# neuphonic/neutts-air

Measured on AMD Instinct MI355X. Metric: codec-tokens/s, higher is better.
Workload: dtype bf16

## Files before the change

### neutts-air_amd/csrc/kapi.cpp

```cpp
#include <ntts/dev.h>

#include "../../include/neutts_hip.h"
#include "kernels/attn_prefill.h"
#include "kernels/gemm.h"
#include "kernels/gemv.h"
#include "kernels/norm.h"
#include "kernels/sample.h"
#include "kernels/score.h"

#include <string.h>

#include <vector>

using namespace ntts;

extern "C" int ntts_k_gemm_bf16(const void* A, int64_t lda, const void* W, const void* bias, void* C, int64_t ldc,
                                int32_t M, int32_t N, int32_t K, int32_t variant) {
    if (!A || !W || !C || M < 1 || N < 1 || K < 64 || (K % 64) || (lda % 8) || (ldc % 8)) return NTTS_EINVAL;
    GemmArgs a{};
    a.X = (const bf16_t*)A; a.ldx = lda; a.W = (const bf16_t*)W; a.ldw = K; a.bias = (const bf16_t*)bias;
    a.out = C; a.ldo = ldc; a.M = M; a.N = N; a.K = K;
    if (variant == 0) variant = M > 64 ? 1 : 2;
    if (variant == 1) NTTS_GEMM_L(EPI_BF16, a, 1, (hipStream_t)0);
    else if (variant == 2) NTTS_GEMM_S(EPI_BF16, a, 1, (hipStream_t)0);
    else if (variant == 4) NTTS_GEMM_XL(EPI_BF16, a, 1, (hipStream_t)0);
    else if (variant == 5) gemm_launch<4, 4, 4, EPI_BF16, 4, 0, 32>(a, 1, (hipStream_t)0);
    else if (variant == 6) gemm_launch<2, 2, 4, EPI_BF16, 3, 0, 32>(a, 1, (hipStream_t)0);
    else if (variant == 7) gemm_launch<4, 3, 4, EPI_BF16, 2, 0, 64, false, false, 6>(a, 1, (hipStream_t)0);
    else if (variant == 8) gemm_launch<4, 3, 5, EPI_BF16, 2>(a, 1, (hipStream_t)0);
    else if (variant == 9) gemm_launch<4, 2, 5, EPI_BF16, 2>(a, 1, (hipStream_t)0);
    else if (variant == 3) {
        if (bias || (N % 16) || ldc != N) return NTTS_EINVAL;
        const int ks = 4, ns = gemm_nsplit(K, ks);
        float* slabs = nullptr;
        if (hipMalloc((void**)&slabs, (size_t)ns * M * N * sizeof(float)) != hipSuccess) return NTTS_ENOMEM;
        a.out = slabs; a.ldo = N;
        NTTS_GEMM_S(EPI_SPLITK, a, ks, (hipStream_t)0);
        NormArgs n{};
        n.slabs = slabs; n.nslab = ns; n.slab_rows = M; n.resid_out = (bf16_t*)C; n.M = M; n.H = N;
        add_rmsnorm_launch(n, (hipStream_t)0);
        if (hipDeviceSynchronize() != hipSuccess) { hipFree(slabs); return NTTS_EHIP; }
        hipFree(slabs);
    } else return NTTS_EINVAL;
    if (hipDeviceSynchronize() != hipSuccess) return NTTS_EHIP;
    return hipGetLastError() == hipSuccess ? NTTS_OK : NTTS_EHIP;
}

NTTS_KERNEL(256) void fp8_quantize_kernel(const float* in, unsigned char* out, long n, float inv_scale) {
    const long i = ((long)blockIdx.x * 256 + threadIdx.x) * 2;
    if (i + 1 < n) { const unsigned short q = f2fp8x2(in[i] * inv_scale, in[i + 1] * inv_scale); out[i] = (unsigned char)(q & 0xff); out[i + 1] = (unsigned char)(q >> 8); }
    else if (i < n) out[i] = f2fp8c(in[i] * inv_scale);
}
extern "C" int ntts_k_fp8_quantize(const float* in_dev, void* out_dev, int64_t n, float inv_scale) {
    if (!in_dev || !out_dev || n < 1) return NTTS_EINVAL;
    NTTS_LAUNCH((fp8_quantize_kernel), dim3((unsigned)((n + 511) / 512)), dim3(256), (hipStream_t)0, in_dev, (unsigned char*)out_dev, (long)n, inv_scale);
    if (hipDeviceSynchronize() != hipSuccess) return NTTS_EHIP;
    return hipGetLastError() == hipSuccess ? NTTS_OK : NTTS_EHIP;
}
extern "C" int ntts_k_gemm_fp8(const void* A, const void* W, const float* wscale, float xscale, const void* bias, void* C,
                               int32_t M, int32_t N, int32_t K, int32_t variant) {
    if (!A || !W || !wscale || !C || M < 1 || N < 1 || K < 128 || (K % 128) || (N % 8)) return NTTS_EINVAL;
    GemmArgs a{};
    a.X = (const bf16_t*)A; a.ldx = K; a.W = (const bf16_t*)W; a.ldw = K; a.bias = (const bf16_t*)bias;
    a.out = C; a.ldo = N; a.M = M; a.N = N; a.K = K; a.wscale = wscale; a.xscale = xscale;
    if (variant == 2) gemm_launch<4, 1, 1, EPI_BF16, 4, 0, 64, false, true>(a, 1, (hipStream_t)0);
    else if (variant == 4) gemm_launch<4, 4, 4, EPI_BF16, 2, 0, 64, false, true>(a, 1, (hipStream_t)0);
    else gemm_launch<2, 2, 4, EPI_BF16, 2, 0, 64, false, true>(a, 1, (hipStream_t)0);
    if (hipDeviceSynchronize() != hipSuccess) return NTTS_EHIP;
    return hipGetLastError() == hipSuccess ? NTTS_OK : NTTS_EHIP;
}

extern "C" int ntts_k_rmsnorm_bf16(const void* x, const void* w, void* y, int32_t rows, int32_t cols, float eps) {
    if (!x || !w || !y || rows < 1 || cols < 8 || (cols % 8) || cols > 2048) return NTTS_EINVAL;
    NormArgs n{};
    n.o_bf16 = (const bf16_t*)x; n.norm_w = (const bf16_t*)w; n.normed_out = (bf16_t*)y; n.M = rows; n.H = cols; n.eps = eps;
    add_rmsnorm_launch(n, (hipStream_t)0);
    if (hipDeviceSynchronize() != hipSuccess) return NTTS_EHIP;
    return hipGetLastError() == hipSuccess ? NTTS_OK : NTTS_EHIP;
}

NTTS_KERNEL(256) void membw_copy_kernel(const u32x4* src, u32x4* dst, long n) {
    for (long i = (long)blockIdx.x * 256 + threadIdx.x; i < n; i += (long)gridDim.x * 256) dst[i] = src[i];
}

extern "C" int ntts_k_membw(size_t bytes, int32_t iters, double* gbps) {
    if (!gbps || bytes < 4096 || iters < 1) return NTTS_EINVAL;
    void *a = nullptr, *b = nullptr;
    if (hipMalloc(&a, bytes) != hipSuccess || hipMalloc(&b, bytes) != hipSuccess) { if (a) hipFree(a); return NTTS_ENOMEM; }
    hipMemset(a, 1, bytes);
    hipEvent_t e0, e1;
    hipEventCreate(&e0); hipEventCreate(&e1);
    const long n = bytes / 16;
    NTTS_LAUNCH((membw_copy_kernel), dim3(2048), dim3(256), (hipStream_t)0, (const u32x4*)a, (u32x4*)b, n);
    hipEventRecord(e0, 0);
    for (int i = 0; i < iters; ++i) NTTS_LAUNCH((membw_copy_kernel), dim3(2048), dim3(256), (hipStream_t)0, (const u32x4*)a, (u32x4*)b, n);
    hipEventRecord(e1, 0);
    hipEventSynchronize(e1);
    float ms = 0;
    hipEventElapsedTime(&ms, e0, e1);
    *gbps = ms > 0 ? 2.0 * (double)(n * 16) * iters / (ms * 1e-3) / 1e9 : 0;
    hipEventDestroy(e0); hipEventDestroy(e1);
    hipFree(a); hipFree(b);
    return hipDeviceSynchronize() == hipSuccess ? NTTS_OK : NTTS_EHIP;
}

NTTS_KERNEL(64) void empty_kernel(int* p) { if (p && threadIdx.x == 12345) *p = 0; }
NTTS_KERNEL(256) void prefetch_kernel(const u32x4* src, long n16, int* sink) {
    unsigned int acc = 0;
    for (long i = (long)blockIdx.x * 256 + threadIdx.x; i < n16; i += (long)gridDim.x * 256) acc ^= src[i][0];
    if (acc == 0x12345678u && sink) *sink = 1;
}

NTTS_KERNEL(256) void random_fill_kernel(bf16_t* dst, long n, unsigned int seed) {
    for (long i = (long)blockIdx.x * 256 + threadIdx.x; i < n; i += (long)gridDim.x * 256) {
        unsigned int h = (unsigned int)i * 0x9e3779b1u + seed;
        h ^= h >> 15; h *= 0x2c1b3c6du; h ^= h >> 12; h *= 0x297a2d39u; h ^= h >> 15;
        dst[i] = (bf16_t)(((h & 1u) << 15) | ((120u + ((h >> 1) & 7u)) << 7) | ((h >> 4) & 0x7fu));
    }
}

template <int WM, int WN, int TM, int NS, int BK = 64>
static void probe_launch(const GemmArgs& a, int ks, int abl) {
    constexpr int EPI = EPI_BF16;
    switch (abl) {
        case 1: gemm_launch<WM, WN, TM, EPI, NS, 1, BK>(a, ks, 0); break;
        case 2: gemm_launch<WM, WN, TM, EPI, NS, 2, BK>(a, ks, 0); break;
        case 3: gemm_launch<WM, WN, TM, EPI, NS, 3, BK>(a, ks, 0); break;
        case 4: gemm_launch<WM, WN, TM, EPI, NS, 4, BK>(a, ks, 0); break;
        case 7: gemm_launch<WM, WN, TM, EPI, NS, 7, BK>(a, ks, 0); break;
        default: gemm_launch<WM, WN, TM, EPI, NS, 0, BK>(a, ks, 0); break;
    }
}

static void probe_dispatch(int config, const GemmArgs& a, int ks, int abl) {
    switch (config) {
        case 0: NTTS_LAUNCH((empty_kernel), dim3(256), dim3(64), (hipStream_t)0, (int*)nullptr); break;
        case 10: probe_launch<4, 1, 1, 2>(a, ks, abl); break;
        case 11: probe_launch<4, 1, 1, 3>(a, ks, abl); break;
        case 12: probe_launch<4, 1, 1, 4>(a, ks, abl); break;
        case 13: probe_launch<4, 1, 1, 6>(a, ks, abl); break;
        case 20: probe_launch<2, 1, 1, 4>(a, ks, abl); break;
        case 21: probe_launch<2, 1, 2, 4>(a, ks, abl); break;
        case 22: probe_launch<1, 1, 4, 4>(a, ks, abl); break;
        case 23: probe_launch<2, 2, 2, 3>(a, ks, abl); break;
        case 24: probe_launch<4, 2, 1, 3>(a, ks, abl); break;
        case 25: probe_launch<8, 1, 1, 3>(a, ks, abl); break;
        case 26: probe_launch<4, 1, 2, 3>(a, ks, abl); break;
        case 30: probe_launch<2, 2, 4, 2>(a, ks, abl); break;
        case 31: probe_launch<2, 2, 4, 3>(a, ks, abl); break;
        case 40: probe_launch<4, 2, 4, 2>(a, ks, abl); break;
        case 41: probe_launch<2, 4, 4, 2>(a, ks, abl); break;
        case 42: probe_launch<4, 4, 4, 2>(a, ks, abl); break;
        case 43: probe_launch<4, 2, 4, 3>(a, ks, abl); break;
        case 44: probe_launch<2, 2, 8, 2>(a, ks, abl); break;
        case 45: probe_launch<2, 4, 8, 2>(a, ks, abl); break;
        case 46: probe_launch<4, 4, 4, 4, 32>(a, ks, abl); break;
        case 47: probe_launch<4, 4, 4, 3, 32>(a, ks, abl); break;
        case 48: probe_launch<2, 4, 8, 4, 32>(a, ks, abl); break;
        case 49: probe_launch<2, 2, 4, 4, 32>(a, ks, abl); break;
        case 50: probe_launch<4, 1, 4, 3>(a, ks, abl); break;
        case 51: probe_launch<8, 1, 2, 3>(a, ks, abl); break;
        case 52: probe_launch<8, 1, 2, 2>(a, ks, abl); break;
        case 53: probe_launch<8, 2, 2, 2>(a, ks, abl); break;
        case 54: probe_launch<4, 2, 2, 3>(a, ks, abl); break;
        case 55: probe_launch<4, 4, 5, 2>(a, ks, abl); break;
        case 57: probe_launch<2, 4, 10, 2>(a, ks, abl); break;
        case 58: probe_launch<2, 4, 12, 2>(a, ks, abl); break;
        case 59: probe_launch<4, 3, 5, 2>(a, ks, abl); break;
        case 60: probe_launch<4, 2, 5, 2>(a, ks, abl); break;
        case 56: probe_launch<4, 4, 6, 2>(a, ks, abl); break;
        default: break;
    }
}

extern "C" int ntts_k_gemm_probe(int32_t M, int32_t N, int32_t K, int32_t config, int32_t abl, int32_t copies, int32_t iters,
                                 double* us) {
    if (!us || M < 1 || N < 16 || K < 64 || (K % 64) || copies < 1 || iters < 1) return NTTS_EINVAL;
    bf16_t *X = nullptr, *W = nullptr, *C = nullptr;
    const size_t wn = (size_t)N * K;
    if (hipMalloc((void**)&X, (size_t)M * K * 2) != hipSuccess || hipMalloc((void**)&W, wn * 2 * copies) != hipSuccess ||
        hipMalloc((void**)&C, (size_t)M * N * 2) != hipSuccess)
        return NTTS_ENOMEM;
    hipMemset(X, 0x11, (size_t)M * K * 2);
    hipMemset(W, 0x22, wn * 2 * copies);
    if (abl & 32) {
        NTTS_LAUNCH((random_fill_kernel), dim3(2048), dim3(256), (hipStream_t)0, X, (long)M * K, 0x9e3779b9u);
        NTTS_LAUNCH((random_fill_kernel), dim3(2048), dim3(256), (hipStream_t)0, W, (long)(wn * copies), 0x85ebca6bu);
    }
    hipEvent_t e0, e1;
    hipEventCreate(&e0); hipEventCreate(&e1);
    const int ks = config >= 1000 ? config / 1000 : 1;
    config %= 1000;
    const bool pf = (abl & 8) != 0;
    const int tile_major = (abl & 16) ? 1 : 0;
    const bool x_ktm = (abl & 64) != 0;
    abl &= 7;
    auto run = [&](int i) {
        if (pf) NTTS_LAUNCH((prefetch_kernel), dim3(256), dim3(256), (hipStream_t)0, (const u32x4*)(W + (size_t)((i + 1) % copies) * wn), (long)(wn / 8), (int*)nullptr);
        GemmArgs a{};
        a.X = X; a.ldx = K; a.W = W + (size_t)(i % copies) * wn; a.ldw = K; a.out = C; a.ldo = N; a.M = M; a.N = N; a.K = K;
        a.w_tile_major = tile_major;
        if (x_ktm) { a.ldx = 64; a.x_kt_stride = (long)M * 128; }
        probe_dispatch(config, a, ks, abl);
    };
    for (int i = 0; i < copies && i < 8; ++i) run(i);
    hipEventRecord(e0, 0);
    for (int i = 0; i < iters; ++i) run(i);
    hipEventRecord(e1, 0);
    hipEventSynchronize(e1);
    float ms = 0;
    hipEventElapsedTime(&ms, e0, e1);
    *us = (double)ms * 1e3 / iters;
    hipEventDestroy(e0); hipEventDestroy(e1);
    hipFree(X); hipFree(W); hipFree(C);
    return hipDeviceSynchronize() == hipSuccess && hipGetLastError() == hipSuccess ? NTTS_OK : NTTS_EHIP;
}

NTTS_KERNEL(64) void mfma_probe_kernel(float* out) {
    const int l = lane_id(), g = l >> 4, c = l & 15;
    for (int probe = 0; probe < 3; ++probe) {
        bf16x8 a, b;
        for (int j = 0; j < 8; ++j) {
            float av, bv;
            if (probe == 0) { av = (g == 0 && j == 0) ? (float)c : 0.f; bv = (g == 0 && j == 0) ? 1.f : 0.f; }
            else if (probe == 1) { av = (g == 0 && j == 0) ? 1.f : 0.f; bv = (g == 0 && j == 0) ? (float)c : 0.f; }
            else { av = (float)(g * 8 + j + 1); bv = (g * 8 + j == (c * 2 + 1) % 32) ? 1.f : 0.f; }
            a[j] = (short)f2bf(av);
            b[j] = (short)f2bf(bv);
        }
        f32x4 d = {0.f, 0.f, 0.f, 0.f};
        d = mfma16(a, b, d);
        for (int r = 0; r < 4; ++r) out[(probe * 64 + l) * 4 + r] = d[r];
    }
}

NTTS_KERNEL(256) void chain_probe_kernel(int* sink) {
    if (threadIdx.x == 0 && sink[blockIdx.x & 1023] == 0x7fffffff) sink[0] = 1;
}
NTTS_KERNEL(256) void chain_touch_kernel(const u32x4* src, u32x4* dst) {
    const long i = (long)blockIdx.x * 256 + threadIdx.x;
    u32x4 v = src[i];
    v[0] += 1;
    dst[i] = v;
}
extern "C" int ntts_k_launch_chain_probe(int32_t n_kernels, int32_t grid, int32_t block, int32_t iters, double* us_per_chain) {
    if (!us_per_chain || n_kernels < 1 || n_kernels > 4096 || grid < 1 || (block != 256 && block != -256) || iters < 1) return NTTS_EINVAL;
    const bool touch = block < 0;
    block = 256;
    if (touch) {
        u32x4 *src = nullptr, *dst = nullptr;
        const size_t per = (size_t)grid * 256, total = per * n_kernels;
        hipStream_t st = nullptr; hipGraph_t g = nullptr; hipGraphExec_t ge = nullptr;
        if (hipMalloc((void**)&src, total * 16) != hipSuccess || hipMalloc((void**)&dst, per * 16) != hipSuccess) { hipFree(src); return NTTS_ENOMEM; }
        hipMemset(src, 1, total * 16);
        int rc = NTTS_EHIP;
        if (hipStreamCreateWithFlags(&st, hipStreamNonBlocking) == hipSuccess && hipStreamBeginCapture(st, hipStreamCaptureModeThreadLocal) == hipSuccess) {
            for (int i = 0; i < n_kernels; ++i) NTTS_LAUNCH((chain_touch_kernel), dim3(grid), dim3(256), st, (const u32x4*)(src + per * i), dst);
            if (hipStreamEndCapture(st, &g) == hipSuccess && g && hipGraphInstantiate(&ge, g, nullptr, nullptr, 0) == hipSuccess) {
                hipEvent_t e0, e1;
                hipEventCreate(&e0); hipEventCreate(&e1);
                for (int i = 0; i < 3; ++i) hipGraphLaunch(ge, st);
                hipEventRecord(e0, st);
                for (int i = 0; i < iters; ++i) hipGraphLaunch(ge, st);
                hipEventRecord(e1, st);
                if (hipEventSynchronize(e1) == hipSuccess) { float ms = 0; hipEventElapsedTime(&ms, e0, e1); *us_per_chain = (double)ms * 1e3 / iters; rc = NTTS_OK; }
                hipEventDestroy(e0); hipEventDestroy(e1);
            }
        }
        if (ge) hipGraphExecDestroy(ge);
        if (g) hipGraphDestroy(g);
        if (st) hipStreamDestroy(st);
        hipFree(src); hipFree(dst);
        (void)hipGetLastError();
        return rc;
    }
    int* sink = nullptr;
    hipStream_t st = nullptr;
    hipGraph_t g = nullptr;
    hipGraphExec_t ge = nullptr;
    if (hipMalloc((void**)&sink, 4096) != hipSuccess) return NTTS_ENOMEM;
    hipMemset(sink, 0, 4096);
    int rc = NTTS_EHIP;
    if (hipStreamCreateWithFlags(&st, hipStreamNonBlocking) == hipSuccess &&
        hipStreamBeginCapture(st, hipStreamCaptureModeThreadLocal) == hipSuccess) {
        for (int i = 0; i < n_kernels; ++i) NTTS_LAUNCH((chain_probe_kernel), dim3(grid), dim3(block), st, sink);
        if (hipStreamEndCapture(st, &g) == hipSuccess && g && hipGraphInstantiate(&ge, g, nullptr, nullptr, 0) == hipSuccess) {
            hipEvent_t e0, e1;
            hipEventCreate(&e0); hipEventCreate(&e1);
            for (int i = 0; i < 3; ++i) hipGraphLaunch(ge, st);
            hipEventRecord(e0, st);
            for (int i = 0; i < iters; ++i) hipGraphLaunch(ge, st);
            hipEventRecord(e1, st);
            if (hipEventSynchronize(e1) == hipSuccess) {
                float ms = 0;
                hipEventElapsedTime(&ms, e0, e1);
                *us_per_chain = (double)ms * 1e3 / iters;
                rc = NTTS_OK;
            }
            hipEventDestroy(e0); hipEventDestroy(e1);
        }
    }
    if (ge) hipGraphExecDestroy(ge);
    if (g) hipGraphDestroy(g);
    if (st) hipStreamDestroy(st);
    hipFree(sink);
    (void)hipGetLastError();
    return rc;
}

NTTS_KERNEL(256) void silu_probe_kernel(const bf16_t* in, bf16_t* out, long n, int variant) {
    const long i = (long)blockIdx.x * 256 + threadIdx.x;
    if (i >= n) return;
    if (variant == 2) {
        const float a = bf2f(in[i]), b = bf2f(in[(i ^ 1) < n ? (i ^ 1) : i]);
        if (a < -86.5f || b < -86.5f) out[i] = f2bf(silu_fast(a));
        else out[i] = f2bf(silu_fast2(f32x2{a, b})[0]);
        return;
    }
    out[i] = f2bf(variant ? silu_fast(bf2f(in[i])) : silu_f(bf2f(in[i])));
}
extern "C" int ntts_k_silu_probe(const void* in_bf16_dev, void* out_bf16_dev, int64_t n, int32_t variant) {
    if (!in_bf16_dev || !out_bf16_dev || n < 1) return NTTS_EINVAL;
// ... 428 lines not shown
```

### neutts-air_amd/csrc/kernels/gemm.h

```cpp
#pragma once
#include <ntts/dev.h>

namespace ntts {

enum GemmEpi {
    EPI_BF16 = 0,
    EPI_SILU_MUL = 1,
    EPI_SPLITK = 2,
    EPI_ARGMAX = 3,
    EPI_BF16_SILU = 4,
    EPI_F32 = 5,
    EPI_RESID = 6,
    EPI_SILU_SPLIT3 = 7,
    EPI_ARGMAX_PEN = 8,
    EPI_ARGMAX_LSE = 9,
    EPI_ARGMAX_PEN_LSE = 10,
    EPI_ARGMAX_LSE_TGT = 11
};
constexpr bool epi_is_argmax(int epi) { return epi == EPI_ARGMAX || epi == EPI_ARGMAX_PEN || epi == EPI_ARGMAX_LSE || epi == EPI_ARGMAX_PEN_LSE || epi == EPI_ARGMAX_LSE_TGT; }
constexpr bool epi_has_pen(int epi) { return epi == EPI_ARGMAX_PEN || epi == EPI_ARGMAX_PEN_LSE; }
constexpr bool epi_has_lse(int epi) { return epi == EPI_ARGMAX_LSE || epi == EPI_ARGMAX_PEN_LSE || epi == EPI_ARGMAX_LSE_TGT; }
constexpr bool epi_has_tgt(int epi) { return epi == EPI_ARGMAX_LSE_TGT; }

struct GemmArgs {
    const bf16_t* X;
    long ldx;
    const bf16_t* W;
    long ldw;
    int w_tile_major;
    const bf16_t* bias;
    const float* bias_f32;
    void* out;
    long ldo;
    int M, N, K;
    int k_tiles_per_split;
    int mblocks, nblocks;
    float* part_val;
    int* part_idx;
    int part_stride;
    const int* mask_eos;
    int eos_col1;
    float* logits;
    long ld_logits;
    bf16_t* logits_bf16;
    long ld_logits_bf16;
    const unsigned int* seen;
    long seen_pitch;
    const float* rep_pen;
    const float* resid;
    long ldr;
    const bf16_t* resid_bf16;
    long ldrb;
    const float* wscale;
    float xscale;
    float out_fp8_inv;
    int xcd_nsplit, xcd_per;
    int xcd_maffine, xcd_xps;
    long x_kt_stride;
    unsigned long long* tl;
    float* part_sum;
    const int* target;
    float* target_val;
};

NTTS_D void gemm_tile_from_linear(int t, int mblocks, int nblocks, int& mb, int& nb) {
    const int GM = 8;
    const int per_group = GM * nblocks;
    const int g = t / per_group;
    const int first_m = g * GM;
    const int gsz = (mblocks - first_m) < GM ? (mblocks - first_m) : GM;
    const int in = t - g * per_group;
    mb = first_m + in % gsz;
    nb = in / gsz;
}

NTTS_D void gemm_tile_coords(int bid, int mblocks, int nblocks, int& mb, int& nb) {
    const int ntiles = mblocks * nblocks;
    const int xcd = bid & 7, idx = bid >> 3;
    const int q = ntiles >> 3, r = ntiles & 7;
    const int t = (xcd < r ? xcd * (q + 1) : r * (q + 1) + (xcd - r) * q) + idx;
    const int GM = 8;
    const int per_group = GM * nblocks;
    const int g = t / per_group;
    const int first_m = g * GM;
    const int gsz = (mblocks - first_m) < GM ? (mblocks - first_m) : GM;
    const int in = t - g * per_group;
    mb = first_m + in % gsz;
    nb = in / gsz;
}

NTTS_D float silu_f(float x) { return x / (1.0f + fexp(-x)); }
NTTS_D float silu_fast(float x) {
    const float ax = __builtin_fminf(__builtin_fabsf(x), 126.0f);
    if (ax > 87.0f && x < 0.f) return silu_f(x);
    const float t = fexp2(-ax * 1.44269504088896340736f);
    const float r = frcp_refined(1.0f + t);
    return x * (x >= 0.f ? r : t * r);
}
typedef __attribute__((ext_vector_type(2))) float f32x2;
NTTS_D f32x2 silu_fast2(f32x2 x) {
    f32x2 ax;
    ax[0] = __builtin_fminf(__builtin_fabsf(x[0]), 126.0f);
    ax[1] = __builtin_fminf(__builtin_fabsf(x[1]), 126.0f);
    const f32x2 e = ax * -1.44269504088896340736f;
    f32x2 t;
    t[0] = fexp2(e[0]);
    t[1] = fexp2(e[1]);
    const f32x2 d = t + 1.0f;
    f32x2 r;
    r[0] = frcp_raw(d[0]);
    r[1] = frcp_raw(d[1]);
    r = __builtin_elementwise_fma(__builtin_elementwise_fma(-d, r, f32x2{1.0f, 1.0f}), r, r);
    const f32x2 tr = t * r;
    f32x2 sg;
    sg[0] = x[0] >= 0.f ? r[0] : tr[0];
    sg[1] = x[1] >= 0.f ? r[1] : tr[1];
    return x * sg;
}
NTTS_D float rep_penalised(float v, float pen) { return rbf(v < 0.f ? v * pen : v / pen); }
NTTS_D void lse_merge(float& mx, float& sum, float omx, float osum) {
    if (omx > mx) { sum = osum + sum * fexp(mx - omx); mx = omx; }
    else if (omx < mx) sum += osum * fexp(omx - mx);
    else sum += osum;
}
NTTS_D float gemm_bias(const GemmArgs& p, int n) { return p.bias_f32 ? p.bias_f32[n] : (p.bias ? bf2f(p.bias[n]) : 0.f); }

template <int TM, int EPI, int WN, bool F8 = false, bool F16 = false>
NTTS_D void gemm_epilogue(const GemmArgs& p, f32x4 (&acc)[TM][4], int mrow0, int n0, int wn, int nb, int split) {
    const int lane = lane_id();
    const int g = lane >> 4, l15 = lane & 15;
    const int nb16 = n0 + wn * 64 + g * 16;
    float sc[4][4];
    if constexpr (F8) {
#pragma unroll
        for (int j = 0; j < 4; ++j)
#pragma unroll
            for (int r = 0; r < 4; ++r) {
                const int n = nb16 + j * 4 + r;
                sc[j][r] = p.xscale * p.wscale[n < p.N ? n : p.N - 1];
            }
        if constexpr (EPI != EPI_BF16) {
#pragma unroll
            for (int a = 0; a < TM; ++a)
#pragma unroll
                for (int j = 0; j < 4; ++j)
#pragma unroll
                    for (int r = 0; r < 4; ++r) acc[a][j][r] *= sc[j][r];
        }
    }
#pragma unroll
    for (int a = 0; a < TM; ++a) {
        const int m = mrow0 + a * 16 + l15;
        const bool mok = m < p.M;
        if constexpr (EPI == EPI_BF16 || EPI == EPI_BF16_SILU) {
            alignas(16) bf16_t o[16];
#pragma unroll
            for (int j = 0; j < 4; ++j)
#pragma unroll
                for (int r = 0; r < 4; ++r) {
                    const int n = nb16 + j * 4 + r;
                    float v = acc[a][j][r];
                    if constexpr (F8 && EPI == EPI_BF16) v = __builtin_fmaf(v, sc[j][r], n < p.N ? gemm_bias(p, n) : 0.f);
                    else if (n < p.N) v += gemm_bias(p, n);
                    if constexpr (EPI == EPI_BF16_SILU) v = silu_fast(v);
                    o[j * 4 + r] = f2op<F16>(v);
                }
            if (mok) {
                bf16_t* dst = (bf16_t*)p.out + (long)m * p.ldo + nb16;
                if (nb16 + 16 <= p.N) {
                    *(u32x4*)dst = *(u32x4*)&o[0];
                    *(u32x4*)(dst + 8) = *(u32x4*)&o[8];
                } else {
                    for (int e = 0; e < 16; ++e)
                        if (nb16 + e < p.N) dst[e] = o[e];
                }
            }
        } else if constexpr (EPI == EPI_SILU_SPLIT3) {
            alignas(16) bf16_t hi[16], lo[16];
#pragma unroll
            for (int j = 0; j < 4; ++j)
#pragma unroll
                for (int r = 0; r < 4; ++r) {
                    const int n = nb16 + j * 4 + r;
                    float v = acc[a][j][r];
                    if (n < p.N) v += gemm_bias(p, n);
                    v = silu_fast(v);
                    hi[j * 4 + r] = f2bf(v);
                    lo[j * 4 + r] = f2bf(v - bf2f(hi[j * 4 + r]));
                }
            if (mok) {
                bf16_t* dst = (bf16_t*)p.out + (long)m * p.ldo + nb16;
                if (nb16 + 16 <= p.N) {
                    *(u32x4*)dst = *(u32x4*)&hi[0];
                    *(u32x4*)(dst + 8) = *(u32x4*)&hi[8];
                    *(u32x4*)(dst + p.N) = *(u32x4*)&lo[0];
                    *(u32x4*)(dst + p.N + 8) = *(u32x4*)&lo[8];
                    *(u32x4*)(dst + 2 * p.N) = *(u32x4*)&hi[0];
                    *(u32x4*)(dst + 2 * p.N + 8) = *(u32x4*)&hi[8];
                } else {
                    for (int e = 0; e < 16; ++e)
                        if (nb16 + e < p.N) { dst[e] = hi[e]; dst[p.N + e] = lo[e]; dst[2 * p.N + e] = hi[e]; }
                }
            }
        } else if constexpr (EPI == EPI_RESID) {
            if (mok) {
                const bf16_t* rs = p.resid_bf16 + (long)m * p.ldrb + nb16;
                bf16_t* dst = (bf16_t*)p.out + (long)m * p.ldo + nb16;
                if (nb16 + 16 <= p.N) {
                    alignas(16) bf16_t rr[16], o[16];
                    *(u32x4*)&rr[0] = *(const u32x4*)rs;
                    *(u32x4*)&rr[8] = *(const u32x4*)(rs + 8);
#pragma unroll
                    for (int j = 0; j < 4; ++j)
#pragma unroll
                        for (int r = 0; r < 4; ++r)
                            o[j * 4 + r] = f2bf(bf2f(rr[j * 4 + r]) + rbf(acc[a][j][r] + gemm_bias(p, nb16 + j * 4 + r)));
// ... 157 lines not shown
                p.part_idx[pi] = bidx;
                if constexpr (epi_has_lse(EPI)) p.part_sum[pi] = lsum;
            }
        }
    }
}

template <int TM, int TN, int EPI, int WN>
NTTS_D void gemm_epilogue_nat(const GemmArgs& p, f32x4 (&acc)[TM][TN], int mrow0, int nw0, int wn, int nb) {
    const int lane = lane_id();
    const int g = lane >> 4, l15 = lane & 15;
#pragma unroll
    for (int a = 0; a < TM; ++a) {
        const int m = mrow0 + a * 16 + l15;
        const bool mok = m < p.M;
        if constexpr (EPI == EPI_BF16) {
#pragma unroll
            for (int j = 0; j < TN; ++j) {
                const int n4 = nw0 + j * 16 + g * 4;
                alignas(8) bf16_t o[4];
#pragma unroll
                for (int r = 0; r < 4; ++r) o[r] = f2bf(acc[a][j][r] + (n4 + r < p.N ? gemm_bias(p, n4 + r) : 0.f));
                if (mok) {
                    bf16_t* dst = (bf16_t*)p.out + (long)m * p.ldo + n4;
                    if (n4 + 4 <= p.N) *(u32x2*)dst = *(u32x2*)&o[0];
                    else for (int e = 0; e < 4; ++e) if (n4 + e < p.N) dst[e] = o[e];
                }
            }
        } else if constexpr (epi_is_argmax(EPI)) {
            float best = -INFINITY;
            int bidx = 0x7fffffff;
            const int meos = (mok && p.mask_eos) ? p.mask_eos[m] : 0;
            if constexpr (epi_has_pen(EPI)) {
                static_assert(TN % 2 == 0, "whole bitmap words per wave tile");
                const float pen = mok ? p.rep_pen[m] : 1.0f;
                unsigned int sw[TN / 2], any = 0;
#pragma unroll
                for (int q = 0; q < TN / 2; ++q) sw[q] = 0;
                if (pen != 1.0f) {
                    const unsigned int* sp = p.seen + (long)m * p.seen_pitch + (nw0 >> 5);
#pragma unroll
                    for (int q = 0; q < TN / 2; ++q) { sw[q] = sp[q]; any |= sw[q]; }
                }
                if (any) {
#pragma unroll
                    for (int j = 0; j < TN; ++j)
#pragma unroll
                        for (int r = 0; r < 4; ++r)
                            if ((sw[j >> 1] >> ((j & 1) * 16 + g * 4 + r)) & 1u) acc[a][j][r] = rep_penalised(rbf(acc[a][j][r]), pen);
                }
            }
            int tgt = -1;
            if constexpr (epi_has_tgt(EPI)) { if (mok) tgt = p.target[m]; }
#pragma unroll
            for (int j = 0; j < TN; ++j) {
                alignas(8) bf16_t lo[4];
#pragma unroll
                for (int r = 0; r < 4; ++r) {
                    const int n = nw0 + j * 16 + g * 4 + r;
                    float v = rbf(acc[a][j][r]);
                    if (meos && n == (p.eos_col1 > 0 ? p.eos_col1 - 1 : meos - 1)) v = -INFINITY;
                    lo[r] = f2bf(v);
                    if constexpr (epi_has_tgt(EPI)) { if (n == tgt) p.target_val[m] = v; }
                    if (n < p.N) {
                        if (mok && p.logits) p.logits[(long)m * p.ld_logits + n] = v;
                        if (v > best) { best = v; bidx = n; }
                    }
                    if constexpr (epi_has_lse(EPI)) acc[a][j][r] = n < p.N ? v : -INFINITY;
                }
                if (p.logits_bf16 && mok) {
                    const int n4 = nw0 + j * 16 + g * 4;
                    bf16_t* dst = p.logits_bf16 + (long)m * p.ld_logits_bf16 + n4;
                    if (n4 + 4 <= p.N) *(u32x2*)dst = *(u32x2*)&lo[0];
                    else for (int e = 0; e < 4; ++e) if (n4 + e < p.N) dst[e] = lo[e];
                }
            }
            float lsum = 0.f;
            if constexpr (epi_has_lse(EPI)) {
                if (best > -INFINITY) {
#pragma unroll
                    for (int j = 0; j < TN; ++j)
#pragma unroll
                        for (int r = 0; r < 4; ++r) lsum += fexp(acc[a][j][r] - best);
                }
            }
#pragma unroll
            for (int sh = 16; sh <= 32; sh <<= 1) {
                const float ov = shfl_xor(best, sh);
                const int oi = shfl_xor(bidx, sh);
                if constexpr (epi_has_lse(EPI)) {
                    const float os = shfl_xor(lsum, sh);
                    float mx = best;
                    lse_merge(mx, lsum, ov, os);
                }
                if (ov > best || (ov == best && oi < bidx)) { best = ov; bidx = oi; }
            }
            if (mok && g == 0) {
                const long pi = (long)m * p.part_stride + nb * WN + wn;
                p.part_val[pi] = best;
                p.part_idx[pi] = bidx;
                if constexpr (epi_has_lse(EPI)) p.part_sum[pi] = lsum;
            }
        } else {
            static_assert(epi_is_argmax(EPI) || EPI == EPI_BF16, "epilogues of the natural-order tile");
        }
    }
}

template <int WM, int WN, int TM, int EPI, int NS, int ABL = 0, int BK = 64, bool WNT = false, bool F8 = false, int TN = 4, bool F16 = false>
NTTS_KERNEL(WM * WN * 64) void gemm_kernel(GemmArgs p) {
    static_assert(!F16 || (!F8 && TN == 4 && (EPI == EPI_BF16 || EPI == EPI_BF16_SILU || EPI == EPI_F32)), "fp16 operands: codec GEMMs");
    static_assert(BK == 64 || BK == 32, "ring slot K extent");
    static_assert(!F8 || BK == 64, "fp8: one ring slot = 128-byte rows");
    static_assert(TN == 4 || ((epi_is_argmax(EPI) || EPI == EPI_BF16) && !F8 && BK == 64), "natural-order tile: lm_head / prefill QKV, bf16");
    constexpr int ESZ = F8 ? 1 : 2;
    constexpr int CW = TN * 16;
    constexpr int BM = WM * TM * 16, BN = WN * CW, NW = WM * WN;
    constexpr int ROWS = BM + BN;
    constexpr int KC = BK / 8;
    constexpr int RPI = 64 / KC;
    static_assert(ROWS % RPI == 0, "whole loader instructions");
    constexpr int NINST = ROWS / RPI;
    constexpr int SPT = 64 / BK;
    constexpr int PER_WAVE = (NINST + NW - 1) / NW;
    constexpr bool EVEN = NINST % NW == 0;
    static_assert(NS >= 2 && (NS - 2) * PER_WAVE <= 63, "vmcnt range");
    NTTS_SHARED bf16_t lds[NS * ROWS * BK];
    auto swz = [](int rho) { return BK == 64 ? (rho >> 1) & 7 : (rho >> 2) & 3; };

    const int lane = lane_id(), wave = wave_id();
    const int wm = wave / WN, wn = wave % WN;
    const int g = lane >> 4, l15 = lane & 15;
    int mb, nb, split = blockIdx.y;
    if (p.xcd_maffine > 0) {
        const int xcd = blockIdx.x & 7, j = blockIdx.x >> 3;
        const int wi = (xcd % p.xcd_xps) + p.xcd_xps * j;
        if (wi >= p.nblocks * p.xcd_maffine) return;
        mb = xcd / p.xcd_xps;
        nb = wi % p.nblocks;
        split = wi / p.nblocks;
    } else if (p.xcd_nsplit) {
        const int xcd = blockIdx.x & 7, j = blockIdx.x >> 3, xps = 8 / p.xcd_nsplit;
        split = xcd / xps;
        const int t = (xcd % xps) * p.xcd_per + j;
        if (t >= p.mblocks * p.nblocks) return;
        gemm_tile_from_linear(t, p.mblocks, p.nblocks, mb, nb);
    } else {
        gemm_tile_coords(blockIdx.x, p.mblocks, p.nblocks, mb, nb);
    }
    const long tlb = ((long)blockIdx.y * gridDim.x + blockIdx.x) * 16;
    auto mark = [&](int slot) { if (p.tl && wave == 0 && lane == 0) p.tl[tlb + slot] = now_ticks(); };
    mark(0);
    const int m0 = mb * BM, n0 = nb * BN;
    const int ktiles = F8 ? p.K >> 7 : p.K >> 6;
    const int kt0 = split * p.k_tiles_per_split * SPT;
    int nk = ktiles - split * p.k_tiles_per_split;
    if (nk > p.k_tiles_per_split) nk = p.k_tiles_per_split;
    nk *= SPT;

    const char* src[PER_WAVE];
#pragma unroll
    for (int i = 0; i < PER_WAVE; ++i) {
        const int inst = (EVEN || wave + i * NW < NINST) ? wave + i * NW : 0;
        const int rho = inst * RPI + lane / KC;
        const int c = (lane % KC) ^ swz(rho);
        if (rho < BM) {
            int m = m0 + rho;
            if (m > p.M - 1) m = p.M - 1;
            src[i] = (const char*)p.X + (long)m * p.ldx * ESZ + c * 16;
        } else {
            const int q = rho - BM;
            const int wq = q >> 6, j = (q >> 4) & 3, i16 = q & 15;
            int n = TN == 4 ? n0 + wq * 64 + (i16 >> 2) * 16 + j * 4 + (i16 & 3) : n0 + q;
            if (n > p.N - 1) n = p.N - 1;
            src[i] = p.w_tile_major ? (const char*)p.W + (long)(n >> 6) * 64 * p.K * ESZ + (n & 63) * 128 + c * 16
                                    : (const char*)p.W + (long)n * p.ldw * ESZ + c * 16;
        }
    }
    const long xstep = p.x_kt_stride > 0 ? p.x_kt_stride : BK * 2;
    const long wstep = p.w_tile_major ? 8192 : xstep;
    auto stage = [&](int kt, int buf) {
        if constexpr (ABL & 2) return;
#pragma unroll
        for (int i = 0; i < PER_WAVE; ++i) {
            const int inst = wave + i * NW;
            if (!EVEN && inst >= NINST) continue;
            const bool is_w = (inst * RPI) >= BM;
            const char* g = src[i] + (long)(kt0 + kt) * (is_w ? wstep : xstep);
            bf16_t* l = lds + buf * (ROWS * BK) + inst * 512;
            if (WNT && is_w) glds16_nt(g, l); else glds16(g, l);
        }
    };

    f32x4 acc[TM][TN];
#pragma unroll
    for (int a = 0; a < TM; ++a)
#pragma unroll
        for (int j = 0; j < TN; ++j) acc[a][j] = f32x4{0.f, 0.f, 0.f, 0.f};

    int xoff[TM], woff[TN], xsw[TM], wsw[TN];
#pragma unroll
    for (int a = 0; a < TM; ++a) {
        const int rho = wm * TM * 16 + a * 16 + l15;
        xoff[a] = rho * BK;
        xsw[a] = swz(rho);
    }
#pragma unroll
    for (int j = 0; j < TN; ++j) {
        const int rho = BM + wn * CW + j * 16 + l15;
        woff[j] = rho * BK;
        wsw[j] = swz(rho);
    }
    const bool full_share = EVEN || wave + (PER_WAVE - 1) * NW < NINST;

#pragma unroll
    for (int s = 0; s < NS - 1; ++s)
        if (s < nk) stage(s, s);
    mark(1);
    int buf = 0;
    for (int kt = 0; kt < nk; ++kt) {
        if (kt + NS - 2 < nk) {
            if (full_share) wait_vmem_le<(NS - 2) * PER_WAVE>(); else wait_vmem_le<(NS - 2) * (PER_WAVE - 1)>();
        } else wait_vmem();
        sync_keep_dma();
        if (kt == 0) mark(2);
        if (kt + NS - 1 < nk) stage(kt + NS - 1, buf == 0 ? NS - 1 : buf - 1);
        const bf16_t* base = lds + buf * (ROWS * BK);
        buf = buf + 1 == NS ? 0 : buf + 1;
        if constexpr (ABL & 1) continue;
#pragma unroll
        for (int ks = 0; ks < BK / 32; ++ks) {
            const int c = ks * 4 + g;
            bf16x8 xb[TM], wa[TN];
#pragma unroll
            for (int a = 0; a < TM; ++a) xb[a] = ld16<bf16x8>(base + xoff[a] + ((c ^ xsw[a]) << 3));
#pragma unroll
            for (int j = 0; j < TN; ++j) wa[j] = ld16<bf16x8>(base + woff[j] + ((c ^ wsw[j]) << 3));
#pragma unroll
            for (int a = 0; a < TM; ++a)
#pragma unroll
                for (int j = 0; j < TN; ++j) {
                    if constexpr (F8) {
                        const i64x2 w2 = __builtin_bit_cast(i64x2, wa[j]), x2 = __builtin_bit_cast(i64x2, xb[a]);
                        acc[a][j] = mfma16_fp8(w2[0], x2[0], acc[a][j]);
                        acc[a][j] = mfma16_fp8(w2[1], x2[1], acc[a][j]);
                    } else {
                        acc[a][j] = mfma16_op<F16>(wa[j], xb[a], acc[a][j]);
                    }
                }
        }
    }

    if constexpr (ABL & 4) {
        if (acc[0][0][0] != 12345.678f) return;
    }
    if (p.tl && wave == 0 && lane == 0) p.tl[tlb + 3] = now_ticks() + (acc[0][0][0] == 1.2345e30f ? 1 : 0);
    if constexpr (TN == 4) gemm_epilogue<TM, EPI, WN, F8, F16>(p, acc, m0 + wm * TM * 16, n0, wn, nb, split);
    else gemm_epilogue_nat<TM, TN, EPI, WN>(p, acc, m0 + wm * TM * 16, n0 + wn * CW, wn, nb);
    if (p.tl) { mark(4); wait_vmem(); mark(5); }
}





struct GemmShape { int BM, BN, WN; };

template <int WM, int WN, int TM, int EPI, int NS = 2, int ABL = 0, int BK = 64, bool WNT = false, bool F8 = false, int TN = 4, bool F16 = false>
inline void gemm_launch(GemmArgs p, int ksplit, hipStream_t s) {
    constexpr int BM = WM * TM * 16, BN = WN * TN * 16;
    p.mblocks = (p.M + BM - 1) / BM;
    p.nblocks = (p.N + BN - 1) / BN;
    const int ktiles = p.K / (F8 ? 128 : 64);
    if (ksplit < 1) ksplit = 1;
    if (ksplit > ktiles) ksplit = ktiles;
    p.k_tiles_per_split = (ktiles + ksplit - 1) / ksplit;
    const int nsplit = (ktiles + p.k_tiles_per_split - 1) / p.k_tiles_per_split;
    if constexpr (epi_is_argmax(EPI)) p.part_stride = p.nblocks * WN;
    if (EPI == EPI_SPLITK && p.xcd_maffine == -1 && (p.mblocks == 1 || p.mblocks == 2 || p.mblocks == 4 || p.mblocks == 8)) {
        p.xcd_maffine = nsplit;
        p.xcd_xps = 8 / p.mblocks;
        p.xcd_nsplit = 0;
        const int per_xcd = (p.nblocks * nsplit + p.xcd_xps - 1) / p.xcd_xps;
        NTTS_LAUNCH((gemm_kernel<WM, WN, TM, EPI, NS, ABL, BK, WNT, F8, TN, F16>), dim3(8 * per_xcd), dim3(WM * WN * 64), s, p);
        return;
    }
    p.xcd_maffine = 0;
    if (EPI == EPI_SPLITK && p.xcd_nsplit == -1 && (nsplit == 2 || nsplit == 4 || nsplit == 8)) {
        p.xcd_nsplit = nsplit;
        const int xps = 8 / nsplit, tiles = p.mblocks * p.nblocks;
        p.xcd_per = (tiles + xps - 1) / xps;
        NTTS_LAUNCH((gemm_kernel<WM, WN, TM, EPI, NS, ABL, BK, WNT, F8, TN, F16>), dim3(8 * p.xcd_per), dim3(WM * WN * 64), s, p);
        return;
    }
    p.xcd_nsplit = 0;
    NTTS_LAUNCH((gemm_kernel<WM, WN, TM, EPI, NS, ABL, BK, WNT, F8, TN, F16>), dim3(p.mblocks * p.nblocks, nsplit), dim3(WM * WN * 64), s, p);
}

#define NTTS_GEMM_XL(EPI, p, ks, s) ::ntts::gemm_launch<4, 4, 4, EPI, 2>(p, ks, s)
#define NTTS_GEMM_BIG(EPI, p, s) do { \
    const long txl_ = (long)(((p).M + 255) / 256) * (((p).N + 255) / 256), tl_ = (long)(((p).M + 127) / 128) * (((p).N + 127) / 128); \
    if ((p).N >= 256 && txl_ >= 140) NTTS_GEMM_XL(EPI, p, 1, s); else if (tl_ >= 240) NTTS_GEMM_L(EPI, p, 1, s); else NTTS_GEMM_S(EPI, p, 1, s); } while (0)
#define NTTS_GEMM_L(EPI, p, ks, s) ::ntts::gemm_launch<2, 2, 4, EPI, 2>(p, ks, s)
#define NTTS_GEMM_BIG_F16(EPI, p, s) do { \
    const long txl_ = (long)(((p).M + 255) / 256) * (((p).N + 255) / 256), tl_ = (long)(((p).M + 127) / 128) * (((p).N + 127) / 128); \
    if ((p).N >= 256 && txl_ >= 140) ::ntts::gemm_launch<4, 4, 4, EPI, 2, 0, 64, false, false, 4, true>(p, 1, s); \
    else if (tl_ >= 240) ::ntts::gemm_launch<2, 2, 4, EPI, 2, 0, 64, false, false, 4, true>(p, 1, s); \
    else ::ntts::gemm_launch<4, 1, 1, EPI, 4, 0, 64, false, false, 4, true>(p, 1, s); } while (0)
#define NTTS_GEMM_S(EPI, p, ks, s) ::ntts::gemm_launch<4, 1, 1, EPI, 4>(p, ks, s)

template <int EPI>
inline void lm_head_launch_epi(const GemmArgs& a, int head_tile, bool fp8, hipStream_t s) {
    switch (head_tile) {
        case 0:
            if (fp8) gemm_launch<4, 1, 1, EPI, 4, 0, 64, false, true>(a, 1, s);
            else gemm_launch<4, 1, 1, EPI, 4>(a, 1, s);
            break;
        case 4: gemm_launch<4, 3, 4, EPI, 2, 0, 64, true, false, 6>(a, 1, s); break;
        case 3: gemm_launch<4, 3, 5, EPI, 2, 0, 64, true>(a, 1, s); break;
        case 2:
            if (fp8) gemm_launch<4, 4, 4, EPI, 2, 0, 64, true, true>(a, 1, s);
            else gemm_launch<4, 4, 4, EPI, 2, 0, 64, true>(a, 1, s);
            break;
        default:
            if (fp8) gemm_launch<2, 2, 4, EPI, 2, 0, 64, false, true>(a, 1, s);
            else gemm_launch<2, 2, 4, EPI, 2>(a, 1, s);
    }
}
inline void lm_head_launch(const GemmArgs& a, int head_tile, bool fp8, hipStream_t s) {
    if (a.target) {
        lm_head_launch_epi<EPI_ARGMAX_LSE_TGT>(a, head_tile, fp8, s);
    } else if (a.part_sum) {
        if (a.seen) lm_head_launch_epi<EPI_ARGMAX_PEN_LSE>(a, head_tile, fp8, s);
        else lm_head_launch_epi<EPI_ARGMAX_LSE>(a, head_tile, fp8, s);
    } else if (a.seen) lm_head_launch_epi<EPI_ARGMAX_PEN>(a, head_tile, fp8, s);
    else lm_head_launch_epi<EPI_ARGMAX>(a, head_tile, fp8, s);
}
inline long seen_pitch_for(int N) { return ((long)N + 288 + 31) / 32 / 4 * 4 + 4; }

inline int gemm_nsplit(int K, int ksplit, int ktile = 64) {
    const int ktiles = K / ktile;
    if (ksplit < 1) ksplit = 1;
    if (ksplit > ktiles) ksplit = ktiles;
    const int per = (ktiles + ksplit - 1) / ksplit;
    return (ktiles + per - 1) / per;
}

}
```

Before: 186,400.

## Use half-width tile specialization for last N block in XL GEMM

For the 4x4x4 XL GEMM configuration, blocks covering the final 128 or fewer columns of N run a specialized path. Each wave computes a 32-row by 64-column sub-tile over only half the W columns, and stages one fewer load per wave, so no work is wasted on out-of-range columns. The compute body is rewrapped in a generic lambda templated on tile rows and loads per wave. A new variant 10 and extra probe configs allow disabling the path or comparing against it. It adds code size and register pressure, and it assumes the LDS layout still matches when fewer instructions are staged.

```diff
diff --git a/neutts-air_amd/csrc/kapi.cpp b/neutts-air_amd/csrc/kapi.cpp
--- a/neutts-air_amd/csrc/kapi.cpp
+++ b/neutts-air_amd/csrc/kapi.cpp
@@ -29,6 +29,7 @@
     else if (variant == 7) gemm_launch<4, 3, 4, EPI_BF16, 2, 0, 64, false, false, 6>(a, 1, (hipStream_t)0);
     else if (variant == 8) gemm_launch<4, 3, 5, EPI_BF16, 2>(a, 1, (hipStream_t)0);
     else if (variant == 9) gemm_launch<4, 2, 5, EPI_BF16, 2>(a, 1, (hipStream_t)0);
+    else if (variant == 10) { a.no_half_block = 1; NTTS_GEMM_XL(EPI_BF16, a, 1, (hipStream_t)0); }
     else if (variant == 3) {
         if (bias || (N % 16) || ldc != N) return NTTS_EINVAL;
         const int ks = 4, ns = gemm_nsplit(K, ks);
@@ -119,16 +120,16 @@
     }
 }
 
-template <int WM, int WN, int TM, int NS, int BK = 64>
+template <int WM, int WN, int TM, int NS, int BK = 64, int TN = 4>
 static void probe_launch(const GemmArgs& a, int ks, int abl) {
     constexpr int EPI = EPI_BF16;
     switch (abl) {
-        case 1: gemm_launch<WM, WN, TM, EPI, NS, 1, BK>(a, ks, 0); break;
-        case 2: gemm_launch<WM, WN, TM, EPI, NS, 2, BK>(a, ks, 0); break;
-        case 3: gemm_launch<WM, WN, TM, EPI, NS, 3, BK>(a, ks, 0); break;
-        case 4: gemm_launch<WM, WN, TM, EPI, NS, 4, BK>(a, ks, 0); break;
-        case 7: gemm_launch<WM, WN, TM, EPI, NS, 7, BK>(a, ks, 0); break;
-        default: gemm_launch<WM, WN, TM, EPI, NS, 0, BK>(a, ks, 0); break;
+        case 1: gemm_launch<WM, WN, TM, EPI, NS, 1, BK, false, false, TN>(a, ks, 0); break;
+        case 2: gemm_launch<WM, WN, TM, EPI, NS, 2, BK, false, false, TN>(a, ks, 0); break;
+        case 3: gemm_launch<WM, WN, TM, EPI, NS, 3, BK, false, false, TN>(a, ks, 0); break;
+        case 4: gemm_launch<WM, WN, TM, EPI, NS, 4, BK, false, false, TN>(a, ks, 0); break;
+        case 7: gemm_launch<WM, WN, TM, EPI, NS, 7, BK, false, false, TN>(a, ks, 0); break;
+        default: gemm_launch<WM, WN, TM, EPI, NS, 0, BK, false, false, TN>(a, ks, 0); break;
     }
 }
 
@@ -168,6 +169,8 @@
         case 58: probe_launch<2, 4, 12, 2>(a, ks, abl); break;
         case 59: probe_launch<4, 3, 5, 2>(a, ks, abl); break;
         case 60: probe_launch<4, 2, 5, 2>(a, ks, abl); break;
+        case 61: probe_launch<4, 3, 4, 2>(a, ks, abl); break;
+        case 62: probe_launch<4, 3, 4, 2, 64, 6>(a, ks, abl); break;
         case 56: probe_launch<4, 4, 6, 2>(a, ks, abl); break;
         default: break;
     }
diff --git a/neutts-air_amd/csrc/kernels/gemm.h b/neutts-air_amd/csrc/kernels/gemm.h
--- a/neutts-air_amd/csrc/kernels/gemm.h
+++ b/neutts-air_amd/csrc/kernels/gemm.h
@@ -61,7 +61,9 @@
     float* part_sum;
     const int* target;
     float* target_val;
+    int no_half_block;
 };
+template <int V> struct gemm_ic { static constexpr int value = V; };
 
 NTTS_D void gemm_tile_from_linear(int t, int mblocks, int nblocks, int& mb, int& nb) {
     const int GM = 8;
@@ -525,6 +527,9 @@
     auto mark = [&](int slot) { if (p.tl && wave == 0 && lane == 0) p.tl[tlb + slot] = now_ticks(); };
     mark(0);
     const int m0 = mb * BM, n0 = nb * BN;
+    constexpr bool HALF_OK = WM == 4 && WN == 4 && TM == 4 && TN == 4 && BK == 64 && !F8 && !epi_is_argmax(EPI);
+    bool half = false;
+    if constexpr (HALF_OK) half = !p.no_half_block && n0 + 128 >= p.N;
     const int ktiles = F8 ? p.K >> 7 : p.K >> 6;
     const int kt0 = split * p.k_tiles_per_split * SPT;
     int nk = ktiles - split * p.k_tiles_per_split;
@@ -552,10 +557,10 @@
     }
     const long xstep = p.x_kt_stride > 0 ? p.x_kt_stride : BK * 2;
     const long wstep = p.w_tile_major ? 8192 : xstep;
-    auto stage = [&](int kt, int buf) {
+    auto stage = [&](int kt, int buf, auto npw_) {
         if constexpr (ABL & 2) return;
 #pragma unroll
-        for (int i = 0; i < PER_WAVE; ++i) {
+        for (int i = 0; i < decltype(npw_)::value; ++i) {
             const int inst = wave + i * NW;
             if (!EVEN && inst >= NINST) continue;
             const bool is_w = (inst * RPI) >= BM;
@@ -565,73 +570,81 @@
         }
     };
 
-    f32x4 acc[TM][TN];
-#pragma unroll
-    for (int a = 0; a < TM; ++a)
-#pragma unroll
-        for (int j = 0; j < TN; ++j) acc[a][j] = f32x4{0.f, 0.f, 0.f, 0.f};
-
-    int xoff[TM], woff[TN], xsw[TM], wsw[TN];
-#pragma unroll
-    for (int a = 0; a < TM; ++a) {
-        const int rho = wm * TM * 16 + a * 16 + l15;
-        xoff[a] = rho * BK;
-        xsw[a] = swz(rho);
-    }
-#pragma unroll
-    for (int j = 0; j < TN; ++j) {
-        const int rho = BM + wn * CW + j * 16 + l15;
-        woff[j] = rho * BK;
-        wsw[j] = swz(rho);
-    }
-    const bool full_share = EVEN || wave + (PER_WAVE - 1) * NW < NINST;
-
-#pragma unroll
-    for (int s = 0; s < NS - 1; ++s)
-        if (s < nk) stage(s, s);
-    mark(1);
-    int buf = 0;
-    for (int kt = 0; kt < nk; ++kt) {
-        if (kt + NS - 2 < nk) {
-            if (full_share) wait_vmem_le<(NS - 2) * PER_WAVE>(); else wait_vmem_le<(NS - 2) * (PER_WAVE - 1)>();
-        } else wait_vmem();
-        sync_keep_dma();
-        if (kt == 0) mark(2);
-        if (kt + NS - 1 < nk) stage(kt + NS - 1, buf == 0 ? NS - 1 : buf - 1);
-        const bf16_t* base = lds + buf * (ROWS * BK);
-        buf = buf + 1 == NS ? 0 : buf + 1;
-        if constexpr (ABL & 1) continue;
-#pragma unroll
-        for (int ks = 0; ks < BK / 32; ++ks) {
-            const int c = ks * 4 + g;
-            bf16x8 xb[TM], wa[TN];
-#pragma unroll
-            for (int a = 0; a < TM; ++a) xb[a] = ld16<bf16x8>(base + xoff[a] + ((c ^ xsw[a]) << 3));
-#pragma unroll
-            for (int j = 0; j < TN; ++j) wa[j] = ld16<bf16x8>(base + woff[j] + ((c ^ wsw[j]) << 3));
-#pragma unroll
-            for (int a = 0; a < TM; ++a)
-#pragma unroll
-                for (int j = 0; j < TN; ++j) {
-                    if constexpr (F8) {
-                        const i64x2 w2 = __builtin_bit_cast(i64x2, wa[j]), x2 = __builtin_bit_cast(i64x2, xb[a]);
-                        acc[a][j] = mfma16_fp8(w2[0], x2[0], acc[a][j]);
-                        acc[a][j] = mfma16_fp8(w2[1], x2[1], acc[a][j]);
-                    } else {
-                        acc[a][j] = mfma16_op<F16>(wa[j], xb[a], acc[a][j]);
+    auto run = [&](auto tme_, auto npw_, const int xrow0, const int wne) {
+        constexpr int TME = decltype(tme_)::value, NPW = decltype(npw_)::value;
+        f32x4 acc[TME][TN];
+#pragma unroll
+        for (int a = 0; a < TME; ++a)
+#pragma unroll
+            for (int j = 0; j < TN; ++j) acc[a][j] = f32x4{0.f, 0.f, 0.f, 0.f};
+
+        int xoff[TME], woff[TN], xsw[TME], wsw[TN];
+#pragma unroll
+        for (int a = 0; a < TME; ++a) {
+            const int rho = xrow0 + a * 16 + l15;
+            xoff[a] = rho * BK;
+            xsw[a] = swz(rho);
+        }
+#pragma unroll
+        for (int j = 0; j < TN; ++j) {
+            const int rho = BM + wne * CW + j * 16 + l15;
+            woff[j] = rho * BK;
+            wsw[j] = swz(rho);
+        }
+        const bool full_share = NPW < PER_WAVE || EVEN || wave + (PER_WAVE - 1) * NW < NINST;
+
+#pragma unroll
+        for (int s = 0; s < NS - 1; ++s)
+            if (s < nk) stage(s, s, npw_);
+        mark(1);
+        int buf = 0;
+        for (int kt = 0; kt < nk; ++kt) {
+            if (kt + NS - 2 < nk) {
+                if (full_share) wait_vmem_le<(NS - 2) * NPW>(); else wait_vmem_le<(NS - 2) * (NPW - 1)>();
+            } else wait_vmem();
+            sync_keep_dma();
+            if (kt == 0) mark(2);
+            if (kt + NS - 1 < nk) stage(kt + NS - 1, buf == 0 ? NS - 1 : buf - 1, npw_);
+            const bf16_t* base = lds + buf * (ROWS * BK);
+            buf = buf + 1 == NS ? 0 : buf + 1;
+            if constexpr (ABL & 1) continue;
+#pragma unroll
+            for (int ks = 0; ks < BK / 32; ++ks) {
+                const int c = ks * 4 + g;
+                bf16x8 xb[TME], wa[TN];
+#pragma unroll
+                for (int a = 0; a < TME; ++a) xb[a] = ld16<bf16x8>(base + xoff[a] + ((c ^ xsw[a]) << 3));
+#pragma unroll
+                for (int j = 0; j < TN; ++j) wa[j] = ld16<bf16x8>(base + woff[j] + ((c ^ wsw[j]) << 3));
+#pragma unroll
+                for (int a = 0; a < TME; ++a)
+#pragma unroll
+                    for (int j = 0; j < TN; ++j) {
+                        if constexpr (F8) {
+                            const i64x2 w2 = __builtin_bit_cast(i64x2, wa[j]), x2 = __builtin_bit_cast(i64x2, xb[a]);
+                            acc[a][j] = mfma16_fp8(w2[0], x2[0], acc[a][j]);
+                            acc[a][j] = mfma16_fp8(w2[1], x2[1], acc[a][j]);
+                        } else {
+                            acc[a][j] = mfma16_op<F16>(wa[j], xb[a], acc[a][j]);
+                        }
                     }
-                }
-        }
-    }
-
-    if constexpr (ABL & 4) {
-        if (acc[0][0][0] != 12345.678f) return;
-    }
-    if (p.tl && wave == 0 && lane == 0) p.tl[tlb + 3] = now_ticks() + (acc[0][0][0] == 1.2345e30f ? 1 : 0);
-    if constexpr (TN == 4) gemm_epilogue<TM, EPI, WN, F8, F16>(p, acc, m0 + wm * TM * 16, n0, wn, nb, split);
-    else gemm_epilogue_nat<TM, TN, EPI, WN>(p, acc, m0 + wm * TM * 16, n0 + wn * CW, wn, nb);
-    if (p.tl) { mark(4); wait_vmem(); mark(5); }
-}
+            }
+        }
+
+        if constexpr (ABL & 4) {
+            if (acc[0][0][0] != 12345.678f) return;
+        }
+        if (p.tl && wave == 0 && lane == 0) p.tl[tlb + 3] = now_ticks() + (acc[0][0][0] == 1.2345e30f ? 1 : 0);
+        if constexpr (TN == 4) gemm_epilogue<TME, EPI, WN, F8, F16>(p, acc, m0 + xrow0, n0, wne, nb, split);
+        else gemm_epilogue_nat<TME, TN, EPI, WN>(p, acc, m0 + xrow0, n0 + wne * CW, wne, nb);
+        if (p.tl) { mark(4); wait_vmem(); mark(5); }
+    };
+    if constexpr (HALF_OK) {
+        if (half) { run(gemm_ic<2>{}, gemm_ic<PER_WAVE - 1>{}, (wave >> 1) * 32, wave & 1); return; }
+    }
+    run(gemm_ic<TM>{}, gemm_ic<PER_WAVE>{}, wm * TM * 16, wn);
+}
+
 
 
 
```

New measurement: 186,900, median of 6. No clear change (+0.3%).
